# fenghansen/YOND_public

Measured on NVIDIA B200. Metric: raw_MP_per_s_end_to_end_YOND_denoise, higher is better.
Workload: dtype bf16

## Files before the change

yond_public_b200/csrc/conv_tc.cu:

```cuda
#include "conv_tc.cuh"

#include <mutex>

namespace {

constexpr int kEpiWarps = 16;
constexpr int kThreads = 64 + 32 * kEpiWarps;
constexpr int kMaxStagesA = 8;
constexpr int kMaxStagesB = 8;
constexpr int kMaxT = 4;
static_assert(kMaxT == 4, "conv_tc: the issuer dispatches T in {1, 2, 4}");
constexpr int kMaxNT = 256;
constexpr int kCta2MinNT = 128;
constexpr int kMaxTabStages = 64;

struct FastDiv {
  uint32_t mul, shr, d;
};
__host__ FastDiv make_fastdiv(uint32_t d) {
  FastDiv f{0u, 0u, d};
  if (d > 1) {
    uint32_t lg = 0;
    while ((1u << lg) < d) ++lg;
    const uint32_t pw = 31 + lg;
    f.mul = (uint32_t)(((1ull << pw) + d - 1) / d);
    f.shr = pw - 32;
  }
  return f;
}
__device__ __forceinline__ uint32_t fdiv(uint32_t n, const FastDiv& f) { return f.d == 1 ? n : (__umulhi(n, f.mul) >> f.shr); }

struct TcParams {
  int B, H, W;
  int TW, TH, NB, T;
  int t_along_h;
  int tiles_h, tiles_w, tiles_b, tiles_n;
  int NT;
  int N;
  int Cout;
  int CB;
  int ncb0, ncb1;
  int mode;
  int wres;
  int SA, SB;
  uint32_t a_stage_bytes, a_tx_bytes, b_stage_bytes;
  uint32_t sub_off, sbo, tap_r_off;
  uint32_t smem_b_off, smem_bar_off, smem_epi_off;
  int tmem_cols;
  uint32_t b2_stage_bytes, b2_off;
  int cta2;
  int acc_stages;
  FastDiv fd_tiles_n, fd_tiles_w, fd_tiles_h, fd_cout;
  int lg_nchunk;
  uint32_t t_off;
  int epi_split;
  int epi_fixed;
  int paired;
  int cvec;
  uint32_t cmask;
  const float* bias;
  const float* scale;
  const float* shift;
  int act;
  float slope;
  const bf16* res;
  bf16* out0;
  bf16* out1;
  const float* tail_w;
  const float* tail_b;
  const float* tail_z;
  const float* tail_ub;
  float* tail_y;
  int tail_res;
  uint32_t smem_tail_off;
};

struct TcMaps {
  CUtensorMap a[8];
  CUtensorMap w;
  CUtensorMap w2;
};

__device__ __forceinline__ uint32_t smem_u32(const void* p) { return (uint32_t)__cvta_generic_to_shared(p); }

__device__ __forceinline__ void mbar_init(uint32_t bar, uint32_t count) {
  asm volatile("mbarrier.init.shared::cta.b64 [%0], %1;" ::"r"(bar), "r"(count) : "memory");
}
__device__ __forceinline__ void mbar_expect_tx(uint32_t bar, uint32_t bytes) {
  asm volatile("mbarrier.arrive.expect_tx.shared::cta.b64 _, [%0], %1;" ::"r"(bar), "r"(bytes) : "memory");
}
__device__ __forceinline__ void mbar_arrive(uint32_t bar) {
  asm volatile("mbarrier.arrive.shared::cta.b64 _, [%0];" ::"r"(bar) : "memory");
}
__device__ __forceinline__ void mbar_wait(uint32_t bar, uint32_t parity) {
  uint32_t done = 0;
  long long t0 = 0;
  for (uint32_t it = 0;; ++it) {
    asm volatile(
        "{\n\t.reg .pred p;\n\t"
// ... 84 lines not shown
__device__ __forceinline__ void tmem_alloc_pair(uint32_t smem_dst, uint32_t ncols) {
  asm volatile("tcgen05.alloc.cta_group::2.sync.aligned.shared::cta.b32 [%0], %1;" ::"r"(smem_dst), "r"(ncols) : "memory");
}
__device__ __forceinline__ void tmem_relinquish_pair() {
  asm volatile("tcgen05.relinquish_alloc_permit.cta_group::2.sync.aligned;" ::: "memory");
}
__device__ __forceinline__ void tmem_dealloc_pair(uint32_t taddr, uint32_t ncols) {
  asm volatile("tcgen05.dealloc.cta_group::2.sync.aligned.b32 %0, %1;" ::"r"(taddr), "r"(ncols) : "memory");
}
__device__ __forceinline__ void umma_commit_pair(uint32_t bar) {
  asm volatile("tcgen05.commit.cta_group::2.mbarrier::arrive::one.shared::cluster.multicast::cluster.b64 [%0], %1;" ::"r"(bar),
               "h"((uint16_t)3)
               : "memory");
}

__device__ __forceinline__ void tmem_ld16(uint32_t taddr, uint32_t (&v)[16]) {
  asm volatile(
      "tcgen05.ld.sync.aligned.32x32b.x16.b32 "
      "{%0, %1, %2, %3, %4, %5, %6, %7, %8, %9, %10, %11, %12, %13, %14, %15}, [%16];"
      : "=r"(v[0]), "=r"(v[1]), "=r"(v[2]), "=r"(v[3]), "=r"(v[4]), "=r"(v[5]), "=r"(v[6]), "=r"(v[7]), "=r"(v[8]),
        "=r"(v[9]), "=r"(v[10]), "=r"(v[11]), "=r"(v[12]), "=r"(v[13]), "=r"(v[14]), "=r"(v[15])
      : "r"(taddr)
      : "memory");
}
__device__ __forceinline__ void tmem_ld_wait() { asm volatile("tcgen05.wait::ld.sync.aligned;" ::: "memory"); }

__device__ __forceinline__ uint32_t pack_bf16x2(float a, float b) {
  __nv_bfloat162 h = __floats2bfloat162_rn(a, b);
  return *reinterpret_cast<uint32_t*>(&h);
}
__device__ __forceinline__ float2 unpack_bf16x2(uint32_t u) {
  __nv_bfloat162 h = *reinterpret_cast<__nv_bfloat162*>(&u);
  return __bfloat1622float2(h);
}

__device__ __forceinline__ float fast_silu(float v) {
  float t;
  const float h = 0.5f * v;
  asm("tanh.approx.f32 %0, %1;" : "=f"(t) : "f"(h));
  return fmaf(h, t, h);
}

struct AStage {
  int map;
  int c;
  int dw, dh;
  int ntaps;
  int widx0;
  int sx;
};
__device__ __forceinline__ AStage decode_astage(const TcParams& p, int ai) {
  AStage s;
  s.sx = -1;
  if (p.mode == CONV_3X3_S1) {
    const int src = ai >= p.ncb0;
    s.map = src;
    s.c = (src ? ai - p.ncb0 : ai) * p.CB;
    s.dw = -1;
    s.dh = -1;
    s.ntaps = 9;
    s.widx0 = ai * 9;
  } else if (p.mode == CONV_3X3_S2) {
    int cbg = ai / 9, tap = ai - cbg * 9;
    int r = tap / 3, sx = tap - r * 3;
    int src = cbg >= p.ncb0;
    s.map = src * 4 + (r != 1) * 2 + (sx != 1);
    s.c = (src ? cbg - p.ncb0 : cbg) * p.CB;
    s.dh = (r == 0) ? -1 : 0;
    s.dw = (sx == 0) ? -1 : 0;
    s.ntaps = 1;
    s.widx0 = cbg * 9 + tap;
  } else if (p.mode == CONV_UPSC) {
    s.dw = 0;
    s.dh = 0;
    s.ntaps = 1;
    if (ai < p.ncb0) {
      s.map = 0;
      s.c = ai * p.CB;
      s.widx0 = ai;
    } else {
      const int j = ai - p.ncb0;
      const int q = j / p.ncb1, cb = j - q * p.ncb1;
      s.map = 4 + q;
      s.c = cb * p.CB;
      s.widx0 = cb;
      s.sx = q;
    }
  } else {
    int src = ai >= p.ncb0;
    s.map = src;
    s.c = (src ? ai - p.ncb0 : ai) * p.CB;
    s.dw = 0;
    s.dh = 0;
    s.ntaps = 1;
    s.widx0 = ai;
  }
  return s;
}
__host__ __device__ __forceinline__ int num_astages(const TcParams& p) {
  int ncb = p.ncb0 + p.ncb1;
  if (p.mode == CONV_3X3_S1) return ncb;
  if (p.mode == CONV_UPSC) return p.ncb0 + 4 * p.ncb1;
  return p.mode == CONV_3X3_S2 ? ncb * 9 : ncb;
}
__device__ __forceinline__ int num_wtiles(const TcParams& p) {
  int ncb = p.ncb0 + p.ncb1;
  return (p.mode == CONV_3X3_S1 || p.mode == CONV_3X3_S2) ? ncb * 9 : ncb;
}

struct TileCoord {
  int n0, w0, h0, b0, n_idx;
};
__device__ __forceinline__ TileCoord decode_tile(const TcParams& p, int tile) {
  TileCoord t;
  uint32_t m = fdiv((uint32_t)tile, p.fd_tiles_n);
  t.n_idx = tile - (int)m * p.tiles_n;
  uint32_t m2 = fdiv(m, p.fd_tiles_w);
  const int tw_i = (int)(m - m2 * p.tiles_w);
  const uint32_t m3 = fdiv(m2, p.fd_tiles_h);
  const int th_i = (int)(m2 - m3 * p.tiles_h);
  const int tb_i = (int)m3;
  t.w0 = tw_i * p.TW;
  t.h0 = th_i * p.TH * (p.t_along_h ? p.T : 1);
  t.b0 = tb_i * p.NB * (p.t_along_h ? 1 : p.T);
  t.n0 = t.n_idx * p.NT;
  return t;
}

struct TileSched {
  int first, step, n_units, rank, cta2;
};
template <bool kPair>
__device__ __forceinline__ TileSched make_sched(const TcParams& p, int total_tiles) {
  TileSched s;
  s.cta2 = kPair ? 1 : 0;
  if (kPair) {
    s.rank = (int)cluster_ctarank();
    s.first = (int)blockIdx.x >> 1;
    s.step = (int)gridDim.x >> 1;
    const int m_tiles = total_tiles / p.tiles_n;
    s.n_units = ((m_tiles + 1) >> 1) * p.tiles_n;
  } else {
    s.rank = 0;
    s.first = (int)blockIdx.x;
    s.step = (int)gridDim.x;
    s.n_units = total_tiles;
  }
  return s;
}
__device__ __forceinline__ int sched_tile(const TcParams& p, const TileSched& s, int u) {
  if (!s.cta2) return u;
  const int m2 = (int)fdiv((uint32_t)u, p.fd_tiles_n);
  return (2 * m2 + s.rank) * p.tiles_n + (u - m2 * p.tiles_n);
}

__device__ __forceinline__ void umma_step(uint32_t tmem_d, uint32_t& a_lo, uint32_t a_hi, uint32_t& b_lo, uint32_t b_hi,
// ... 37 lines not shown
    dt += nt;
  }
}
template <int KS, int TT>
__device__ __forceinline__ void issue_tap(uint32_t d_tmem, uint32_t nt, uint32_t a_lo0, uint32_t sub_step, uint32_t b_lo0,
                                          uint32_t a_hi, uint32_t b_hi, uint32_t idesc, uint32_t accum) {
  uint32_t al = a_lo0, dt = d_tmem;
#pragma unroll
  for (int t = 0; t < TT; ++t) {
    uint32_t bl = b_lo0;
#pragma unroll
    for (int k = 0; k < KS; ++k) umma_step(dt, al, a_hi, bl, b_hi, idesc, k ? 1u : accum);
    al += sub_step - 2u * KS;
    dt += nt;
  }
}

template <int K0, int K1, int TT>
__device__ __forceinline__ void issue_tap_range(uint32_t d_tmem, uint32_t nt, uint32_t a_lo0, uint32_t sub_step, uint32_t b_lo0,
                                                uint32_t a_hi, uint32_t b_hi, uint32_t idesc, uint32_t accum) {
  uint32_t al = a_lo0 + 2u * K0, dt = d_tmem;
#pragma unroll
  for (int t = 0; t < TT; ++t) {
    uint32_t bl = b_lo0 + 2u * K0;
#pragma unroll
    for (int k = K0; k < K1; ++k) umma_step(dt, al, a_hi, bl, b_hi, idesc, k > K0 ? 1u : accum);
    al += sub_step - 2u * (K1 - K0);
    dt += nt;
  }
}
template <int TT>
__device__ __forceinline__ void issue_slab_paired(uint32_t d_tmem, uint32_t nt, uint32_t a_stage_lo, uint32_t tap_r16, uint32_t px16,
                                                  uint32_t sub_step, uint32_t b_lo_first, uint32_t b_step16, uint32_t a_hi,
                                                  uint32_t b_hi, uint32_t idesc, uint32_t first_accum) {
#pragma unroll
  for (int r = 0; r < 3; ++r) {
    const uint32_t a0 = a_stage_lo + (uint32_t)r * tap_r16, b0 = b_lo_first + (uint32_t)(r * 3) * b_step16;
    issue_tap_range<2, 4, TT>(d_tmem, nt, a0, sub_step, b0, a_hi, b_hi, idesc, r ? 1u : first_accum);
    issue_tap_range<0, 4, TT>(d_tmem, nt, a0 + px16, sub_step, b0 + b_step16, a_hi, b_hi, idesc, 1u);
    issue_tap_range<0, 2, TT>(d_tmem, nt, a0 + 2u * px16, sub_step, b0 + 2u * b_step16, a_hi, b_hi, idesc, 1u);
  }
}

template <int KS, int TT>
__device__ __forceinline__ void issue_slab_resident(uint32_t d_tmem, uint32_t nt, uint32_t a_stage_lo, uint32_t tap_r16, uint32_t px16,
                                                    uint32_t sub_step, uint32_t b_lo_first, uint32_t b_step16, uint32_t a_hi,
                                                    uint32_t b_hi, uint32_t idesc, uint32_t first_accum) {
#pragma unroll
  for (int r = 0; r < 3; ++r)
#pragma unroll
    for (int sx = 0; sx < 3; ++sx)
      issue_tap_range<0, KS, TT>(d_tmem, nt, a_stage_lo + (uint32_t)r * tap_r16 + (uint32_t)sx * px16, sub_step,
                                 b_lo_first + (uint32_t)(r * 3 + sx) * b_step16, a_hi, b_hi, idesc, (r | sx) ? 1u : first_accum);
}

struct __align__(32) U8 { uint32_t v[8]; };
__device__ __forceinline__ void stg256(void* ptr, const U8& u) {
  asm volatile("st.global.v8.b32 [%0], {%1, %2, %3, %4, %5, %6, %7, %8};" ::"l"(ptr), "r"(u.v[0]), "r"(u.v[1]), "r"(u.v[2]), "r"(u.v[3]),
               "r"(u.v[4]), "r"(u.v[5]), "r"(u.v[6]), "r"(u.v[7])
               : "memory");
}
__device__ __forceinline__ U8 ldg256(const void* ptr) {
  U8 u;
  asm volatile("ld.global.nc.v8.b32 {%0, %1, %2, %3, %4, %5, %6, %7}, [%8];"
               : "=r"(u.v[0]), "=r"(u.v[1]), "=r"(u.v[2]), "=r"(u.v[3]), "=r"(u.v[4]), "=r"(u.v[5]), "=r"(u.v[6]), "=r"(u.v[7])
               : "l"(ptr));
  return u;
}

__device__ __forceinline__ float4 lds_f4(uint32_t addr) {
  float4 v;
  asm volatile("ld.shared.v4.f32 {%0, %1, %2, %3}, [%4];" : "=f"(v.x), "=f"(v.y), "=f"(v.z), "=f"(v.w) : "r"(addr) : "memory");
  return v;
}
__device__ __forceinline__ void sts_f32(uint32_t addr, float v) { asm volatile("st.shared.f32 [%0], %1;" ::"r"(addr), "f"(v) : "memory"); }
__device__ __forceinline__ void sts_u4(uint32_t addr, uint32_t a, uint32_t b, uint32_t c, uint32_t d) {
  asm volatile("st.shared.v4.b32 [%0], {%1, %2, %3, %4};" ::"r"(addr), "r"(a), "r"(b), "r"(c), "r"(d) : "memory");
}
__device__ __forceinline__ uint4 lds_u4(uint32_t addr) {
  uint4 v;
  asm volatile("ld.shared.v4.b32 {%0, %1, %2, %3}, [%4];" : "=r"(v.x), "=r"(v.y), "=r"(v.z), "=r"(v.w) : "r"(addr));
  return v;
}

__device__ __forceinline__ bool epilogue_single_set(const TcParams& p) {
  const int nparts = p.epi_split ? 2 : 4, nchunk = 1 << p.lg_nchunk;
  const int nsets = nchunk > nparts ? nchunk / nparts : 1;
  return p.epi_fixed != 0 && nsets <= 2 && (nsets == 1 || (((uint32_t)(nparts << 4) & p.cmask) == 0u));
}
template <bool kScale, bool kRes, bool kSilu, int kV, bool kPair, bool kRegP = false>
__device__ __forceinline__ void epilogue_loop(const TcParams& p, uint32_t tmem_base, uint32_t acc_full, uint32_t acc_empty, uint32_t ptab,
                                              int warp, int lane, int total_tiles) {
  const TileSched sched = make_sched<kPair>(p, total_tiles);
  const uint32_t acc_empty_remote = kPair ? mapa_shared(acc_empty, 0) : acc_empty;
  const int q = warp & 3;
  const int part4 = (warp - 2) >> 2;
  const bool split = p.epi_split != 0;
  const int grp = split ? (part4 & 1) : 0;
  const int part = split ? (part4 >> 1) : part4;
  const int nparts = split ? 2 : 4;
  const int row = q * 32 + lane;
  const int w_i = row & (p.TW - 1);
  const int g_i = row / p.TW;
  const int dh = g_i / p.NB, db = g_i & (p.NB - 1);
  const int nchunk = 1 << p.lg_nchunk, nchunk_m1 = nchunk - 1, nvis = p.T << p.lg_nchunk;
  const int nsets = nchunk > nparts ? nchunk / nparts : 1;
// ... 306 lines not shown
    mbar_init(w_full, 1);
    fence_barrier_init();
  }
  if (p.tail_w) {
    for (int i = threadIdx.x; i < 132; i += blockDim.x)
      sts_f32(smem_base + p.smem_tail_off + 4 * i, i < 128 ? __ldg(p.tail_w + i) : __ldg(p.tail_b + i - 128));
  }
  if (warp == 1) {
    if (kPair) {
      tmem_alloc_pair(tmem_slot, p.tmem_cols);
      tmem_relinquish_pair();
    } else {
      tmem_alloc(tmem_slot, p.tmem_cols);
      tmem_relinquish();
    }
  }
  tc_fence_before();
  __syncthreads();
  if (kPair) cluster_sync_all();
  tc_fence_after();
  const TileSched sched = make_sched<kPair>(p, total_tiles);
  const bool pair_leader = sched.rank == 0;
  uint32_t tmem_base;
  asm volatile("ld.shared.u32 %0, [%1];" : "=r"(tmem_base) : "r"(tmem_slot));

  if (warp == 0) {
    const uint32_t is_leader = elect_one();
    if (is_leader) {
      tma_prefetch_desc(&maps.w);
      tma_prefetch_desc(&maps.a[0]);
      if (p.wres && p.mode == CONV_UPSC) {
        mbar_expect_tx(w_full, p.ncb0 * p.b_stage_bytes + p.ncb1 * p.b2_stage_bytes);
        for (int i = 0; i < p.ncb0; ++i) tma_load_2d(smem_b + i * p.b_stage_bytes, &maps.w, w_full, 0, i * p.N);
        for (int i = 0; i < p.ncb1; ++i) tma_load_2d(smem_b + p.b2_off + i * p.b2_stage_bytes, &maps.w2, w_full, 0, i * p.Cout);
      } else if (p.wres) {
        const int nwt = num_wtiles(p);
        mbar_expect_tx(w_full, nwt * p.b_stage_bytes);
        for (int i = 0; i < nwt; ++i) tma_load_2d(smem_b + i * p.b_stage_bytes, &maps.w, w_full, 0, i * p.N);
      }
    }
    __syncwarp();
    int sa = 0, pa = 0, sb = 0, pb = 0;
    const uint32_t a_full_sig = kPair ? mapa_shared(a_full, 0) : a_full;
    const uint32_t b_full_sig = kPair ? mapa_shared(b_full, 0) : b_full;
    const uint32_t b_half = kPair ? (uint32_t)(sched.rank * (p.NT / 2)) : 0u;
    for (int u = sched.first; u < sched.n_units; u += sched.step) {
      const TileCoord tc = decode_tile(p, sched_tile(p, sched, u));
      for (int ai = 0; ai < n_ast; ++ai) {
        const AStage s = decode_astage(p, ai);
        mbar_wait(a_empty + 8 * sa, pa ^ 1);
        if (is_leader) {
          if (kPair) {
            if (pair_leader) mbar_expect_tx(a_full + 8 * sa, 2 * p.a_tx_bytes);
            tma_load_4d_pair(smem_a + sa * p.a_stage_bytes, &maps.a[s.map], a_full_sig + 8 * sa, s.c, tc.w0 + s.dw, tc.b0, tc.h0 + s.dh);
          } else {
            mbar_expect_tx(a_full + 8 * sa, p.a_tx_bytes);
            tma_load_4d(smem_a + sa * p.a_stage_bytes, &maps.a[s.map], a_full + 8 * sa, s.c, tc.w0 + s.dw, tc.b0, tc.h0 + s.dh);
          }
        }
        __syncwarp();
        if (++sa == p.SA) { sa = 0; pa ^= 1; }
        if (!p.wres) {
          for (int j = 0; j < s.ntaps; ++j) {
            const int widx = s.widx0 + j;
            mbar_wait(b_empty + 8 * sb, pb ^ 1);
            if (is_leader) {
              if (kPair) {
                if (pair_leader) mbar_expect_tx(b_full + 8 * sb, 2 * p.b_stage_bytes);
                tma_load_2d_pair(smem_b + sb * p.b_stage_bytes, &maps.w, b_full_sig + 8 * sb, 0, widx * p.N + tc.n0 + (int)b_half);
              } else {
                mbar_expect_tx(b_full + 8 * sb, p.b_stage_bytes);
                tma_load_2d(smem_b + sb * p.b_stage_bytes, &maps.w, b_full + 8 * sb, 0, widx * p.N + tc.n0);
              }
            }
            __syncwarp();
            if (++sb == p.SB) { sb = 0; pb ^= 1; }
          }
        }
      }
    }
  } else if (warp == 1) {
    const uint32_t u_tmem = __reduce_max_sync(0xffffffffu, tmem_base);
    const uint32_t u_smem_a = __reduce_max_sync(0xffffffffu, smem_a);
    const uint32_t u_smem_b = __reduce_max_sync(0xffffffffu, smem_b);
    const uint32_t u_bars = __reduce_max_sync(0xffffffffu, bars);
    const uint32_t ua_full = u_bars, ua_empty = ua_full + 8 * kMaxStagesA;
    const uint32_t ub_full = ua_empty + 8 * kMaxStagesA, ub_empty = ub_full + 8 * kMaxStagesB;
    const uint32_t uacc_full = ub_empty + 8 * kMaxStagesB, uacc_empty = uacc_full + 16;
    const uint32_t uw_full = uacc_empty + 16;
    const uint32_t idesc = (1u << 4) | (1u << 7) | (1u << 10) | ((uint32_t)(p.NT >> 3) << 17) | (((kPair ? 256u : 128u) >> 4) << 24);
    const uint32_t idesc_full = idesc;
    const int ksteps = p.CB / 16;
    const uint32_t layout = (row_bytes == 128) ? 2u : 4u;
    const uint32_t a_hi = ((p.sbo >> 4) & 0x3FFFu) | (1u << 14) | (layout << 29);
    const uint32_t b_hi = (((8u * row_bytes) >> 4) & 0x3FFFu) | (1u << 14) | (layout << 29);
    const uint32_t lo_flags = 1u << 16;
    const uint32_t sub_step = p.sub_off >> 4;
    const uint32_t tap_r16 = p.tap_r_off >> 4, px16 = row_bytes >> 4;
    const uint32_t nt = (uint32_t)p.NT;
    const bool leader = elect_one() != 0;
    if (p.wres) mbar_wait(uw_full, 0);
    int sa = 0, pa = 0, sb = 0, pb = 0, as = 0, pacc = 0;
    const bool fast_slab1 = p.wres && p.mode == CONV_3X3_S1 && n_ast == 1 && !kPair;
    if (fast_slab1) {
      const uint32_t b_first = (((u_smem_b) & 0x3FFFFu) >> 4) | lo_flags;
      const uint32_t b_step16 = p.b_stage_bytes >> 4;
      const uint32_t a_bytes = p.a_stage_bytes, acc_cols = (uint32_t)p.T * nt;
      const int SA = p.SA, nacc = p.acc_stages;
      auto run = [&](auto issue) {
        for (int u = sched.first; u < sched.n_units; u += sched.step) {
          mbar_wait(uacc_empty + 8 * as, pacc ^ 1);
          mbar_wait(ua_full + 8 * sa, pa);
          tc_fence_after();
          if (leader) {
            issue(u_tmem + (uint32_t)as * acc_cols, (((u_smem_a + (uint32_t)sa * a_bytes) & 0x3FFFFu) >> 4) | lo_flags);
            umma_commit(ua_empty + 8 * sa);
            umma_commit(uacc_full + 8 * as);
          }
          __syncwarp();
          if (++sa == SA) { sa = 0; pa ^= 1; }
          if (++as == nacc) { as = 0; pacc ^= 1; }
        }
      };
#define YOND_SLAB1(FN) run([&](uint32_t d, uint32_t a_lo) { FN(d, nt, a_lo, tap_r16, px16, sub_step, b_first, b_step16, a_hi, b_hi, idesc, 0u); })
      if (p.paired) {
        if (p.T == 1) YOND_SLAB1((issue_slab_paired<1>));
        else if (p.T == 2) YOND_SLAB1((issue_slab_paired<2>));
        else YOND_SLAB1((issue_slab_paired<4>));
      } else if (ksteps == 4) {
        if (p.T == 1) YOND_SLAB1((issue_slab_resident<4, 1>));
        else if (p.T == 2) YOND_SLAB1((issue_slab_resident<4, 2>));
        else YOND_SLAB1((issue_slab_resident<4, 4>));
      } else {
        if (p.T == 1) YOND_SLAB1((issue_slab_resident<2, 1>));
        else if (p.T == 2) YOND_SLAB1((issue_slab_resident<2, 2>));
        else YOND_SLAB1((issue_slab_resident<2, 4>));
      }
#undef YOND_SLAB1
    }
    const bool fast_tab = p.wres && p.mode != CONV_3X3_S1 && !kPair;
    if (fast_tab) {
      const uint32_t tab = smem_base + p.smem_tail_off;
      for (int ai = lane; ai < n_ast; ai += 32) {
        const AStage s = decode_astage(p, ai);
        uint32_t b_lo0 = (((smem_b + (uint32_t)s.widx0 * p.b_stage_bytes) & 0x3FFFFu) >> 4) | lo_flags;
        uint32_t id = idesc_full, d_off = 0;
        if (p.mode == CONV_UPSC && s.sx >= 0) {
          b_lo0 = (((smem_b + p.b2_off + (uint32_t)s.widx0 * p.b2_stage_bytes) & 0x3FFFFu) >> 4) | lo_flags;
          id = (idesc_full & ~(0x3Fu << 17)) | ((uint32_t)(p.Cout >> 3) << 17);
          d_off = (uint32_t)(s.sx * p.Cout);
        }
        sts_u4(tab + 16u * (uint32_t)ai, b_lo0, id, d_off, 0u);
      }
      __syncwarp();
      const uint32_t a_bytes = p.a_stage_bytes, acc_cols = (uint32_t)p.T * nt;
      const int SA = p.SA, nacc = p.acc_stages;
      auto run = [&](auto issue) {
        for (int u = sched.first; u < sched.n_units; u += sched.step) {
          mbar_wait(uacc_empty + 8 * as, pacc ^ 1);
          const uint32_t d_tile = u_tmem + (uint32_t)as * acc_cols;
          for (int ai = 0; ai < n_ast; ++ai) {
            mbar_wait(ua_full + 8 * sa, pa);
            tc_fence_after();
            if (leader) {
              const uint4 e = lds_u4(tab + 16u * (uint32_t)ai);
              issue(d_tile + e.z, (((u_smem_a + (uint32_t)sa * a_bytes) & 0x3FFFFu) >> 4) | lo_flags, e.x, e.y, ai ? 1u : 0u);
              umma_commit(ua_empty + 8 * sa);
            }
            __syncwarp();
            if (++sa == SA) { sa = 0; pa ^= 1; }
          }
          if (leader) umma_commit(uacc_full + 8 * as);
          __syncwarp();
          if (++as == nacc) { as = 0; pacc ^= 1; }
        }
      };
#define YOND_TAB(KS, TT) run([&](uint32_t d, uint32_t a_lo, uint32_t b_lo, uint32_t id, uint32_t acc) { issue_tap<KS, TT>(d, nt, a_lo, sub_step, b_lo, a_hi, b_hi, id, acc); })
      if (ksteps == 4) {
        if (p.T == 1) YOND_TAB(4, 1);
        else if (p.T == 2) YOND_TAB(4, 2);
        else YOND_TAB(4, 4);
      } else {
        if (p.T == 1) YOND_TAB(2, 1);
        else if (p.T == 2) YOND_TAB(2, 2);
        else YOND_TAB(2, 4);
      }
#undef YOND_TAB
    }
    const bool fast_stream = !p.wres && p.mode == CONV_3X3_S1 && ksteps == 4;
    if (fast_stream && (!kPair || pair_leader)) {
      const uint32_t a_bytes = p.a_stage_bytes, b_bytes = p.b_stage_bytes, acc_cols = (uint32_t)p.T * nt;
      const int SA = p.SA, SB = p.SB, nacc = p.acc_stages;
      auto commit = [&](uint32_t bar) {
        if (kPair) umma_commit_pair(bar);
        else umma_commit(bar);
      };
      auto run = [&](auto issue) {
        for (int u = sched.first; u < sched.n_units; u += sched.step) {
          mbar_wait(uacc_empty + 8 * as, pacc ^ 1);
          const uint32_t d_tile = u_tmem + (uint32_t)as * acc_cols;
          for (int ai = 0; ai < n_ast; ++ai) {
            mbar_wait(ua_full + 8 * sa, pa);
            tc_fence_after();
            if (leader) {
              const uint32_t a_stage_lo = (((u_smem_a + (uint32_t)sa * a_bytes) & 0x3FFFFu) >> 4) | lo_flags;
              int lsb = sb, lpb = pb;
#pragma unroll
              for (int j = 0; j < 9; ++j) {
                const uint32_t r = j / 3, sx = j % 3;
                mbar_wait(ub_full + 8 * lsb, lpb);
                tc_fence_after();
                issue(d_tile, a_stage_lo + r * tap_r16 + sx * px16, (((u_smem_b + (uint32_t)lsb * b_bytes) & 0x3FFFFu) >> 4) | lo_flags,
                      (ai | j) ? 1u : 0u);
                commit(ub_empty + 8 * lsb);
                if (++lsb == SB) { lsb = 0; lpb ^= 1; }
              }
              commit(ua_empty + 8 * sa);
            }
            __syncwarp();
            sb += 9;
            while (sb >= SB) { sb -= SB; pb ^= 1; }
            if (++sa == SA) { sa = 0; pa ^= 1; }
          }
          if (leader) commit(uacc_full + 8 * as);
          __syncwarp();
          if (++as == nacc) { as = 0; pacc ^= 1; }
        }
      };
#define YOND_STREAM(TT)                                                                                                   \
  run([&](uint32_t d, uint32_t a_lo, uint32_t b_lo, uint32_t acc) {                                                      \
    if (kPair) issue_tap_pair<4, TT>(d, nt, a_lo, sub_step, b_lo, a_hi, b_hi, idesc, acc);                               \
    else issue_tap<4, TT>(d, nt, a_lo, sub_step, b_lo, a_hi, b_hi, idesc, acc);                                          \
  })
      if (p.T == 1) YOND_STREAM(1);
      else if (p.T == 2) YOND_STREAM(2);
      else YOND_STREAM(4);
#undef YOND_STREAM
    }
    if (!kPair && !fast_slab1 && !fast_tab && !fast_stream) {
      for (int u = sched.first; u < sched.n_units; u += sched.step) {
        mbar_wait(uacc_empty + 8 * as, pacc ^ 1);
        tc_fence_after();
        const uint32_t d_tmem = u_tmem + (uint32_t)(as * p.T) * nt;
        for (int ai = 0; ai < n_ast; ++ai) {
          const AStage s = decode_astage(p, ai);
          mbar_wait(ua_full + 8 * sa, pa);
          tc_fence_after();
          const uint32_t a_stage_lo = (((u_smem_a + (uint32_t)sa * p.a_stage_bytes) & 0x3FFFFu) >> 4) | lo_flags;
          if (leader && p.wres) {
            const uint32_t b_first = (((u_smem_b + (uint32_t)s.widx0 * p.b_stage_bytes) & 0x3FFFFu) >> 4) | lo_flags;
            const uint32_t b_step16 = p.b_stage_bytes >> 4;
            const uint32_t acc0 = ai ? 1u : 0u;
            if (ksteps == 4) {
              if (p.T == 1) issue_slab_resident<4, 1>(d_tmem, nt, a_stage_lo, tap_r16, px16, sub_step, b_first, b_step16, a_hi, b_hi, idesc, acc0);
              else if (p.T == 2) issue_slab_resident<4, 2>(d_tmem, nt, a_stage_lo, tap_r16, px16, sub_step, b_first, b_step16, a_hi, b_hi, idesc, acc0);
              else issue_slab_resident<4, 4>(d_tmem, nt, a_stage_lo, tap_r16, px16, sub_step, b_first, b_step16, a_hi, b_hi, idesc, acc0);
            } else {
              if (p.T == 1) issue_slab_resident<2, 1>(d_tmem, nt, a_stage_lo, tap_r16, px16, sub_step, b_first, b_step16, a_hi, b_hi, idesc, acc0);
              else if (p.T == 2) issue_slab_resident<2, 2>(d_tmem, nt, a_stage_lo, tap_r16, px16, sub_step, b_first, b_step16, a_hi, b_hi, idesc, acc0);
              else issue_slab_resident<2, 4>(d_tmem, nt, a_stage_lo, tap_r16, px16, sub_step, b_first, b_step16, a_hi, b_hi, idesc, acc0);
            }
            umma_commit(ua_empty + 8 * sa);
          } else if (leader) {
            int lsb = sb, lpb = pb;
            for (int j = 0; j < s.ntaps; ++j) {
              uint32_t r = 0, sx = 0;
              if (p.mode == CONV_3X3_S1) { r = (j >= 3) + (j >= 6); sx = j - r * 3; }
              mbar_wait(ub_full + 8 * lsb, lpb);
              tc_fence_after();
              const uint32_t a_lo0 = a_stage_lo + r * tap_r16 + sx * px16;
              const uint32_t b_lo0 = (((u_smem_b + (uint32_t)lsb * p.b_stage_bytes) & 0x3FFFFu) >> 4) | lo_flags;
              const uint32_t accum = (ai | j) ? 1u : 0u;
              if (ksteps == 4) {
                if (p.T == 1) issue_tap<4, 1>(d_tmem, nt, a_lo0, sub_step, b_lo0, a_hi, b_hi, idesc, accum);
                else if (p.T == 2) issue_tap<4, 2>(d_tmem, nt, a_lo0, sub_step, b_lo0, a_hi, b_hi, idesc, accum);
                else issue_tap<4, 4>(d_tmem, nt, a_lo0, sub_step, b_lo0, a_hi, b_hi, idesc, accum);
              } else {
                if (p.T == 1) issue_tap<2, 1>(d_tmem, nt, a_lo0, sub_step, b_lo0, a_hi, b_hi, idesc, accum);
                else if (p.T == 2) issue_tap<2, 2>(d_tmem, nt, a_lo0, sub_step, b_lo0, a_hi, b_hi, idesc, accum);
                else issue_tap<2, 4>(d_tmem, nt, a_lo0, sub_step, b_lo0, a_hi, b_hi, idesc, accum);
              }
              umma_commit(ub_empty + 8 * lsb);
              if (++lsb == p.SB) { lsb = 0; lpb ^= 1; }
            }
            umma_commit(ua_empty + 8 * sa);
          }
          __syncwarp();
          if (!p.wres) {
            sb += s.ntaps;
            while (sb >= p.SB) { sb -= p.SB; pb ^= 1; }
          }
          if (++sa == p.SA) { sa = 0; pa ^= 1; }
        }
        if (leader) umma_commit(uacc_full + 8 * as);
        __syncwarp();
        if (++as == p.acc_stages) { as = 0; pacc ^= 1; }
      }
    }
  } else {
    const bool silu = p.act == ACT_SILU;
    const uint32_t ptab = smem_base + p.smem_epi_off + (uint32_t)(warp - 2) * 256u;
#define YOND_EPI(S, R, A, V) epilogue_loop<S, R, A, V, kPair>(p, tmem_base, acc_full, acc_empty, ptab, warp, lane, total_tiles)
    const bool few = p.T * (p.NT / 16) <= 8;
    if (!kPair && p.tail_w) {
      const uint32_t tailtab = smem_base + p.smem_tail_off;
      if (p.scale && p.res) epilogue_tail<true, true>(p, tmem_base, acc_full, acc_empty, ptab, tailtab, warp, lane, total_tiles);
      else if (p.scale) epilogue_tail<true, false>(p, tmem_base, acc_full, acc_empty, ptab, tailtab, warp, lane, total_tiles);
      else if (p.res) epilogue_tail<false, true>(p, tmem_base, acc_full, acc_empty, ptab, tailtab, warp, lane, total_tiles);
      else epilogue_tail<false, false>(p, tmem_base, acc_full, acc_empty, ptab, tailtab, warp, lane, total_tiles);
    }
    else if (p.scale && p.res) { if (silu) YOND_EPI(true, true, true, 2); else YOND_EPI(true, true, false, 2); }
    else if (p.scale && epilogue_single_set(p)) {
      if (silu) epilogue_loop<true, false, true, 4, kPair, true>(p, tmem_base, acc_full, acc_empty, ptab, warp, lane, total_tiles);
      else epilogue_loop<true, false, false, 4, kPair, true>(p, tmem_base, acc_full, acc_empty, ptab, warp, lane, total_tiles);
    }
    else if (p.scale) { if (silu) YOND_EPI(true, false, true, 4); else YOND_EPI(true, false, false, 4); }
    else if (p.res && epilogue_single_set(p)) {
#define YOND_EPI_R(A, V) epilogue_loop<false, true, A, V, kPair, true>(p, tmem_base, acc_full, acc_empty, ptab, warp, lane, total_tiles)
      if (few) { if (silu) YOND_EPI_R(true, 2); else YOND_EPI_R(false, 2); }
      else { if (silu) YOND_EPI_R(true, 4); else YOND_EPI_R(false, 4); }
#undef YOND_EPI_R
    }
    else if (p.res) {
// ... 89 lines not shown
  for (int r = 0; r < 3; ++r)
    for (int P = -1; P <= 1; ++P)
      for (int o = 0; o < 2; ++o)
        for (int co = 0; co < 32; ++co)
          for (int i = 0; i < 2; ++i)
            for (int ci = 0; ci < 32; ++ci) {
              const int dx = 2 * P + i - o;
              const float v = (dx >= -1 && dx <= 1) ? w[((size_t)co * 32 + ci) * 9 + r * 3 + (dx + 1)] : 0.f;
              out[((size_t)(r * 3 + P + 1) * 64 + (o * 32 + co)) * 64 + (i * 32 + ci)] = __float2bfloat16_rn(v);
            }
}

int conv_tc_launch(const ConvLayer& Lin, cudaStream_t stream) {
  ConvLayer L = Lin;
  const bool paired = L.wpaired && L.mode == CONV_3X3_S1 && L.Cin0 == 32 && L.Cin1 == 0 && L.Cout == 32 && L.Win % 2 == 0 &&
                      L.res == nullptr && L.tail_w == nullptr;
  if (paired) {
    L.Win /= 2;
    L.Cin0 = 64;
    L.Cout = 64;
    L.wpacked = L.wpaired;
  }
  YOND_REQUIRE(L.Cin0 % 32 == 0 && L.Cin1 % 32 == 0 && L.Cin0 > 0, "conv_tc: Cin must be a multiple of 32 (got %d,%d)",
               L.Cin0, L.Cin1);
  YOND_REQUIRE(L.Cout % 32 == 0, "conv_tc: Cout must be a multiple of 32 (got %d)", L.Cout);
  YOND_REQUIRE((double)L.B * L.Hin * L.Win * ((L.mode == CONVT_2X2 || L.mode == CONV_UPSC) ? 4.0 : 1.0) * L.Cout < 4294967296.0,
               "conv_tc: output of %d x %d x %d x %d elements exceeds the 32-bit offset range; split the batch", L.B, L.Hin, L.Win, L.Cout);
  YOND_REQUIRE(L.scale != nullptr || L.shift == nullptr, "conv_tc: a shift vector needs a scale vector");
  TcParams p{};
  p.mode = L.mode;
  p.B = L.B;
  if (L.mode == CONV_3X3_S2) {
    YOND_REQUIRE(L.Hin % 2 == 0 && L.Win % 2 == 0, "conv_tc: stride-2 conv needs even input dims");
    p.H = L.Hin / 2;
    p.W = L.Win / 2;
  } else {
    p.H = L.Hin;
    p.W = L.Win;
  }
  p.Cout = L.Cout;
  p.paired = paired ? 1 : 0;
  p.cvec = paired ? 32 : L.Cout;
  p.cmask = paired ? 31u : 0xffffffffu;
  const bool convt_like = L.mode == CONVT_2X2 || L.mode == CONV_UPSC;
  p.N = convt_like ? 4 * L.Cout : L.Cout;
  p.CB = conv_tc_channel_block(L.Cin0, L.Cin1);
  p.ncb0 = L.Cin0 / p.CB;
  p.ncb1 = L.Cin1 / p.CB;
  p.NT = p.N < kMaxNT ? p.N : kMaxNT;
  YOND_REQUIRE(p.N % p.NT == 0 && (p.NT & (p.NT - 1)) == 0, "conv_tc: unsupported N=%d", p.N);
  p.tiles_n = p.N / p.NT;
  const uint32_t row_bytes = p.CB * 2;
  const bool conv3 = L.mode == CONV_3X3_S1;

  p.TW = conv3 ? 8 : (p.W > 8 ? 16 : 8);
  const int rows = 128 / p.TW;
  p.TH = pow2_ceil(p.H) < rows ? pow2_ceil(p.H) : rows;
  p.NB = rows / p.TH;
  const int ncb = p.ncb0 + p.ncb1;
  const int nwt = ((L.mode == CONV_3X3_S1 || L.mode == CONV_3X3_S2) ? 9 : 1) * ncb;
  const size_t smem_budget = 227 * 1024 - 2048 - kEpiWarps * 256 - 1024;
  p.b_stage_bytes = (uint32_t)p.NT * row_bytes;
  YOND_REQUIRE(p.b_stage_bytes % 1024 == 0, "conv_tc: weight stage not 1024-aligned");
  size_t wres_bytes = (size_t)nwt * p.b_stage_bytes;
  if (L.mode == CONV_UPSC) {
    YOND_REQUIRE(L.Cin1 == L.Cout && L.src1 != nullptr, "conv_tc: fused up-sampling needs a skip source with Cout channels");
    p.b2_stage_bytes = (uint32_t)L.Cout * row_bytes;
    p.b2_off = (uint32_t)p.ncb0 * p.b_stage_bytes;
    wres_bytes = (size_t)p.b2_off + (size_t)p.ncb1 * p.b2_stage_bytes;
    YOND_REQUIRE(p.tiles_n == 1 && wres_bytes <= 80 * 1024 && p.b2_stage_bytes % 1024 == 0,
                 "conv_tc: fused up-sampling is built for resident weights (Cout <= 64); got Cout=%d", L.Cout);
  }
  p.wres = (p.tiles_n == 1 && wres_bytes <= 80 * 1024) ? 1 : 0;
  YOND_REQUIRE(!p.wres || conv3 || num_astages(p) <= kMaxTabStages, "conv_tc: %d resident-weight stages exceed the stage table (%d)",
               num_astages(p), kMaxTabStages);
  p.cta2 = (conv3 && !p.wres && p.CB == 64 && p.NT >= kCta2MinNT && yond_num_sms() >= 2) ? 1 : 0;
  if (p.cta2) p.b_stage_bytes /= 2;
  int T = 1;
  {
    int tmax = (p.wres || p.cta2) ? 512 / (2 * p.NT) : 512 / p.NT;
    if (tmax > kMaxT) tmax = kMaxT;
    if (p.NB == 1) {
      while (T * 2 <= tmax && (p.H >= p.TH * T * 2 || (conv3 && p.B >= T * 2))) T *= 2;
    } else if (conv3) {
      while (T * 2 <= tmax && p.B >= p.NB * T * 2) T *= 2;
    }
  }
  int slab_w = 0, slab_h = 0, SBt = 0;
  size_t b_region = 0;
  for (;; T /= 2) {
    p.T = T;
    p.t_along_h = (p.H >= p.TH * T) ? 1 : 0;
    const int SH = p.TH * (p.t_along_h ? T : 1);
    SBt = p.NB * (p.t_along_h ? 1 : T);
    p.tiles_w = ceil_div(p.W, p.TW);
    p.tiles_h = ceil_div(p.H, SH);
    p.tiles_b = ceil_div(p.B, SBt);
    slab_w = conv3 ? p.TW + 2 : p.TW;
    slab_h = conv3 ? SH + 2 : SH;
    const uint32_t line = (uint32_t)slab_w * row_bytes;
    p.a_tx_bytes = (uint32_t)slab_h * SBt * line;
    p.a_stage_bytes = (uint32_t)align_up((size_t)p.a_tx_bytes, 1024);
    if (conv3) {
      p.tap_r_off = (uint32_t)SBt * line;
      p.sbo = p.t_along_h ? line : (uint32_t)T * line;
      p.sub_off = p.t_along_h ? (uint32_t)p.TH * line : line;
    } else {
      p.tap_r_off = 0;
      p.sbo = 8u * row_bytes;
      p.sub_off = (uint32_t)p.TH * line;
    }
    if (p.wres) {
      p.SB = 1;
      b_region = wres_bytes;
      p.SA = (int)((smem_budget - b_region) / p.a_stage_bytes);
      if (p.SA > kMaxStagesA) p.SA = kMaxStagesA;
      if (p.SA >= 3 || T == 1) break;
    } else {
      const size_t rest = smem_budget > 2 * (size_t)p.a_stage_bytes ? smem_budget - 2 * (size_t)p.a_stage_bytes : 0;
      p.SB = (int)(rest / p.b_stage_bytes);
      if (p.SB > kMaxStagesB) p.SB = kMaxStagesB;
      b_region = (size_t)p.SB * p.b_stage_bytes;
      p.SA = p.SB > 0 ? (int)((smem_budget - b_region) / p.a_stage_bytes) : 0;
      if (p.SA > kMaxStagesA) p.SA = kMaxStagesA;
      if ((p.SB >= 3 && p.SA >= 2) || T == 1) break;
    }
  }
  YOND_REQUIRE(p.SB >= 1, "conv_tc: not enough shared memory for the weight ring");
  YOND_REQUIRE(p.SA >= 2, "conv_tc: not enough shared memory for the activation pipeline");
  p.smem_b_off = (uint32_t)p.SA * p.a_stage_bytes;
  p.smem_bar_off = (uint32_t)align_up(p.smem_b_off + b_region, 1024);
  p.smem_epi_off = p.smem_bar_off + 512;
  p.smem_tail_off = p.smem_epi_off + kEpiWarps * 256;
  const size_t smem_bytes = p.smem_tail_off + 1024 + 1024;
  p.acc_stages = 2 * p.T * p.NT <= 512 ? 2 : 1;
  p.epi_split = (p.acc_stages == 2 && p.paired) ? 1 : 0;
  p.tmem_cols = p.acc_stages * p.T * p.NT < 32 ? 32 : p.acc_stages * p.T * p.NT;
  YOND_REQUIRE(p.tmem_cols <= 512, "conv_tc: TMEM budget exceeded");

  p.fd_tiles_n = make_fastdiv((uint32_t)p.tiles_n);
  p.fd_tiles_w = make_fastdiv((uint32_t)p.tiles_w);
  p.fd_tiles_h = make_fastdiv((uint32_t)p.tiles_h);
  p.fd_cout = make_fastdiv((uint32_t)p.Cout);
  p.lg_nchunk = 0;
  while ((16 << p.lg_nchunk) < p.NT) ++p.lg_nchunk;
  if (convt_like) p.t_off = (uint32_t)p.TH * 4u * p.W * p.Cout;
  else p.t_off = (p.t_along_h ? (uint32_t)p.TH * p.W : (uint32_t)p.H * p.W) * (uint32_t)p.Cout;
  YOND_REQUIRE(L.act != ACT_LRELU || (L.slope >= 0.f && L.slope <= 1.f), "conv_tc: LeakyReLU slope must be in [0, 1]");
  {
    const int nchunk = p.NT / 16;
    p.epi_fixed = (p.tiles_n == 1 && nchunk <= 4 && p.NB == 1 && (p.T == 1 || p.t_along_h) && !convt_like) ? 1 : 0;
  }
  p.bias = L.bias;
  p.scale = L.scale;
  p.shift = L.shift;
  p.act = L.act;
  p.slope = L.slope;
  p.res = L.res;
  p.out0 = L.out0;
  p.out1 = L.out1;
  if (L.tail_w) {
    YOND_REQUIRE(L.mode == CONV_3X3_S1 && L.Cout == 32 && !paired && p.tiles_n == 1 && p.NT == 32 && p.T <= 4 && !p.cta2 && L.tail_b &&
                     L.tail_y && (L.tail_z || !L.tail_res),
                 "conv_tc: the fused output conv needs a 3x3 layer with 32 output channels");
    p.tail_w = L.tail_w;
    p.tail_b = L.tail_b;
    p.tail_z = L.tail_z;
    p.tail_ub = L.tail_ub;
    p.tail_y = L.tail_y;
    p.tail_res = L.tail_res;
    p.epi_split = 0;
  }

  TcMaps maps;
  memset(&maps, 0, sizeof(maps));
  const bf16* srcs[2] = {L.src0, L.src1};
  const int cins[2] = {L.Cin0, L.Cin1};
  for (int s = 0; s < 2; ++s) {
    if (cins[s] == 0) continue;
    const int C = cins[s];
    if (L.mode == CONV_UPSC && s == 1) {
      for (int ph = 0; ph < 2; ++ph)
        for (int pw = 0; pw < 2; ++pw) {
          const int Wh = 2 * L.Win, Hh = 2 * L.Hin;
          const bf16* base = srcs[s] + ((size_t)ph * Wh + pw) * C;
          int rc = make_act_map(&maps.a[4 + ph * 2 + pw], base, C, L.Win, L.B, L.Hin, (uint64_t)2 * C * 2,
                                (uint64_t)Hh * Wh * C * 2, (uint64_t)2 * Wh * C * 2, p.CB, slab_w, SBt, slab_h);
          if (rc) return rc;
        }
    } else if (L.mode == CONV_3X3_S2) {
      for (int ph = 0; ph < 2; ++ph)
        for (int pw = 0; pw < 2; ++pw) {
          const bf16* base = srcs[s] + ((size_t)ph * L.Win + pw) * C;
          int rc = make_act_map(&maps.a[s * 4 + ph * 2 + pw], base, C, L.Win / 2, L.B, L.Hin / 2, (uint64_t)2 * C * 2,
                                (uint64_t)L.Hin * L.Win * C * 2, (uint64_t)2 * L.Win * C * 2, p.CB, slab_w, SBt, slab_h);
          if (rc) return rc;
        }
    } else {
      int rc = make_act_map(&maps.a[s], srcs[s], C, L.Win, L.B, L.Hin, (uint64_t)C * 2, (uint64_t)L.Hin * L.Win * C * 2,
                            (uint64_t)L.Win * C * 2, p.CB, slab_w, SBt, slab_h);
      if (rc) return rc;
    }
  }
  {
    const size_t rows_a = L.mode == CONV_UPSC ? (size_t)p.ncb0 * p.N : (size_t)nwt * p.N;
    int rc = make_weight_map(&maps.w, L.wpacked, p.CB, rows_a, p.cta2 ? p.NT / 2 : p.NT);
    if (rc) return rc;
    if (L.mode == CONV_UPSC) {
      rc = make_weight_map(&maps.w2, L.wpacked + rows_a * p.CB, p.CB, (size_t)p.ncb1 * L.Cout, L.Cout);
      if (rc) return rc;
    }
  }
  static std::once_flag attr_once;
  static cudaError_t attr_err = cudaSuccess;
  std::call_once(attr_once, [] {
    attr_err = cudaFuncSetAttribute(conv_tc_kernel<false>, cudaFuncAttributeMaxDynamicSharedMemorySize, 227 * 1024);
    if (attr_err == cudaSuccess)
      attr_err = cudaFuncSetAttribute(conv_tc_kernel<true>, cudaFuncAttributeMaxDynamicSharedMemorySize, 227 * 1024);
  });
  if (attr_err != cudaSuccess)
    return yond_set_error(YOND_ERR_CUDA, "cudaFuncSetAttribute(conv_tc_kernel) failed: %s", cudaGetErrorString(attr_err));

  const int total_tiles = p.tiles_b * p.tiles_h * p.tiles_w * p.tiles_n;
  if (p.cta2) {
    const int m_tiles = total_tiles / p.tiles_n;
    const int units = ((m_tiles + 1) / 2) * p.tiles_n;
    int grid = yond_num_sms() & ~1;
    if (grid > 2 * units) grid = 2 * units;
    cudaLaunchConfig_t cfg{};
    cfg.gridDim = dim3((unsigned)grid);
    cfg.blockDim = dim3(kThreads);
    cfg.dynamicSmemBytes = smem_bytes;
    cfg.stream = stream;
    cudaLaunchAttribute attr[1];
    attr[0].id = cudaLaunchAttributeClusterDimension;
    attr[0].val.clusterDim.x = 2;
    attr[0].val.clusterDim.y = 1;
    attr[0].val.clusterDim.z = 1;
    cfg.attrs = attr;
    cfg.numAttrs = 1;
    cudaError_t e = cudaLaunchKernelEx(&cfg, conv_tc_kernel<true>, maps, p);
    if (e != cudaSuccess) return yond_set_error(YOND_ERR_CUDA, "conv_tc: cluster launch failed: %s", cudaGetErrorString(e));
    yond_count_launch(1);
    return YOND_OK;
  }
  int grid = yond_num_sms();
  if (grid > total_tiles) grid = total_tiles;
  conv_tc_kernel<false><<<grid, kThreads, smem_bytes, stream>>>(maps, p);
// ... 4 lines not shown
```

Baseline: 2845.

## Load all four stride-2 parity slabs per channel block and issue 9 taps from smem

Stride-2 3x3 convolutions previously used one activation stage per tap, issuing nine separate TMA loads of shifted parity slabs per channel block. Now each A stage holds all four parity sub-slabs (odd-row ones one row taller, with one extra column), and the MMA issuer walks the nine taps through precomputed smem offsets. The S2 path is also routed through the resident-slab, streaming and 2-CTA paths that S1 already used. This cuts TMA traffic and pipeline stages by roughly nine times. In exchange each stage is larger, which means fewer stages fit in shared memory, and the S2 path is forced to T=1.

```diff
diff --git a/yond_public_b200/csrc/conv_tc.cu b/yond_public_b200/csrc/conv_tc.cu
--- a/yond_public_b200/csrc/conv_tc.cu
+++ b/yond_public_b200/csrc/conv_tc.cu
@@ -45,6 +45,7 @@
   int SA, SB;
   uint32_t a_stage_bytes, a_tx_bytes, b_stage_bytes;
   uint32_t sub_off, sbo, tap_r_off;
+  uint32_t par_off[4], s2_tap16[9];
   uint32_t smem_b_off, smem_bar_off, smem_epi_off;
   int tmem_cols;
   uint32_t b2_stage_bytes, b2_off;
@@ -235,24 +236,14 @@
 __device__ __forceinline__ AStage decode_astage(const TcParams& p, int ai) {
   AStage s;
   s.sx = -1;
-  if (p.mode == CONV_3X3_S1) {
+  if (p.mode == CONV_3X3_S1 || p.mode == CONV_3X3_S2) {
     const int src = ai >= p.ncb0;
-    s.map = src;
+    s.map = p.mode == CONV_3X3_S2 ? src * 4 : src;
     s.c = (src ? ai - p.ncb0 : ai) * p.CB;
     s.dw = -1;
     s.dh = -1;
     s.ntaps = 9;
     s.widx0 = ai * 9;
-  } else if (p.mode == CONV_3X3_S2) {
-    int cbg = ai / 9, tap = ai - cbg * 9;
-    int r = tap / 3, sx = tap - r * 3;
-    int src = cbg >= p.ncb0;
-    s.map = src * 4 + (r != 1) * 2 + (sx != 1);
-    s.c = (src ? cbg - p.ncb0 : cbg) * p.CB;
-    s.dh = (r == 0) ? -1 : 0;
-    s.dw = (sx == 0) ? -1 : 0;
-    s.ntaps = 1;
-    s.widx0 = cbg * 9 + tap;
   } else if (p.mode == CONV_UPSC) {
     s.dw = 0;
     s.dh = 0;
@@ -282,9 +273,8 @@
 }
 __host__ __device__ __forceinline__ int num_astages(const TcParams& p) {
   int ncb = p.ncb0 + p.ncb1;
-  if (p.mode == CONV_3X3_S1) return ncb;
   if (p.mode == CONV_UPSC) return p.ncb0 + 4 * p.ncb1;
-  return p.mode == CONV_3X3_S2 ? ncb * 9 : ncb;
+  return ncb;
 }
 __device__ __forceinline__ int num_wtiles(const TcParams& p) {
   int ncb = p.ncb0 + p.ncb1;
@@ -428,6 +418,14 @@
     for (int sx = 0; sx < 3; ++sx)
       issue_tap_range<0, KS, TT>(d_tmem, nt, a_stage_lo + (uint32_t)r * tap_r16 + (uint32_t)sx * px16, sub_step,
                                  b_lo_first + (uint32_t)(r * 3 + sx) * b_step16, a_hi, b_hi, idesc, (r | sx) ? 1u : first_accum);
+}
+template <int KS>
+__device__ __forceinline__ void issue_slab_s2(uint32_t d_tmem, uint32_t a_stage_lo, const uint32_t (&tap16)[9], uint32_t b_lo_first,
+                                              uint32_t b_step16, uint32_t a_hi, uint32_t b_hi, uint32_t idesc, uint32_t first_accum) {
+#pragma unroll
+  for (int j = 0; j < 9; ++j)
+    issue_tap_range<0, KS, 1>(d_tmem, 0u, a_stage_lo + tap16[j], 0u, b_lo_first + (uint32_t)j * b_step16, a_hi, b_hi, idesc,
+                              j ? 1u : first_accum);
 }
 
 struct __align__(32) U8 { uint32_t v[8]; };
@@ -840,10 +838,18 @@
         if (is_leader) {
           if (kPair) {
             if (pair_leader) mbar_expect_tx(a_full + 8 * sa, 2 * p.a_tx_bytes);
-            tma_load_4d_pair(smem_a + sa * p.a_stage_bytes, &maps.a[s.map], a_full_sig + 8 * sa, s.c, tc.w0 + s.dw, tc.b0, tc.h0 + s.dh);
           } else {
             mbar_expect_tx(a_full + 8 * sa, p.a_tx_bytes);
-            tma_load_4d(smem_a + sa * p.a_stage_bytes, &maps.a[s.map], a_full + 8 * sa, s.c, tc.w0 + s.dw, tc.b0, tc.h0 + s.dh);
+          }
+          auto load_a = [&](uint32_t off, int map, int h) {
+            if (kPair) tma_load_4d_pair(smem_a + sa * p.a_stage_bytes + off, &maps.a[map], a_full_sig + 8 * sa, s.c, tc.w0 + s.dw, tc.b0, h);
+            else tma_load_4d(smem_a + sa * p.a_stage_bytes + off, &maps.a[map], a_full + 8 * sa, s.c, tc.w0 + s.dw, tc.b0, h);
+          };
+          if (p.mode == CONV_3X3_S2) {
+#pragma unroll
+            for (int q = 0; q < 4; ++q) load_a(p.par_off[q], s.map + q, tc.h0 + s.dh + 1 - (q >> 1));
+          } else {
+            load_a(0u, s.map, tc.h0 + s.dh);
           }
         }
         __syncwarp();
@@ -889,7 +895,7 @@
     const bool leader = elect_one() != 0;
     if (p.wres) mbar_wait(uw_full, 0);
     int sa = 0, pa = 0, sb = 0, pb = 0, as = 0, pacc = 0;
-    const bool fast_slab1 = p.wres && p.mode == CONV_3X3_S1 && n_ast == 1 && !kPair;
+    const bool fast_slab1 = p.wres && (p.mode == CONV_3X3_S1 || p.mode == CONV_3X3_S2) && n_ast == 1 && !kPair;
     if (fast_slab1) {
       const uint32_t b_first = (((u_smem_b) & 0x3FFFFu) >> 4) | lo_flags;
       const uint32_t b_step16 = p.b_stage_bytes >> 4;
@@ -911,7 +917,10 @@
         }
       };
 #define YOND_SLAB1(FN) run([&](uint32_t d, uint32_t a_lo) { FN(d, nt, a_lo, tap_r16, px16, sub_step, b_first, b_step16, a_hi, b_hi, idesc, 0u); })
-      if (p.paired) {
+      if (p.mode == CONV_3X3_S2) {
+        if (ksteps == 4) run([&](uint32_t d, uint32_t a_lo) { issue_slab_s2<4>(d, a_lo, p.s2_tap16, b_first, b_step16, a_hi, b_hi, idesc, 0u); });
+        else run([&](uint32_t d, uint32_t a_lo) { issue_slab_s2<2>(d, a_lo, p.s2_tap16, b_first, b_step16, a_hi, b_hi, idesc, 0u); });
+      } else if (p.paired) {
         if (p.T == 1) YOND_SLAB1((issue_slab_paired<1>));
         else if (p.T == 2) YOND_SLAB1((issue_slab_paired<2>));
         else YOND_SLAB1((issue_slab_paired<4>));
@@ -926,7 +935,7 @@
       }
 #undef YOND_SLAB1
     }
-    const bool fast_tab = p.wres && p.mode != CONV_3X3_S1 && !kPair;
+    const bool fast_tab = p.wres && p.mode != CONV_3X3_S1 && p.mode != CONV_3X3_S2 && !kPair;
     if (fast_tab) {
       const uint32_t tab = smem_base + p.smem_tail_off;
       for (int ai = lane; ai < n_ast; ai += 32) {
@@ -975,7 +984,7 @@
       }
 #undef YOND_TAB
     }
-    const bool fast_stream = !p.wres && p.mode == CONV_3X3_S1 && ksteps == 4;
+    const bool fast_stream = !p.wres && (p.mode == CONV_3X3_S1 || p.mode == CONV_3X3_S2) && ksteps == 4;
     if (fast_stream && (!kPair || pair_leader)) {
       const uint32_t a_bytes = p.a_stage_bytes, b_bytes = p.b_stage_bytes, acc_cols = (uint32_t)p.T * nt;
       const int SA = p.SA, SB = p.SB, nacc = p.acc_stages;
@@ -983,7 +992,7 @@
         if (kPair) umma_commit_pair(bar);
         else umma_commit(bar);
       };
-      auto run = [&](auto issue) {
+      auto run = [&](auto issue, auto tap_off) {
         for (int u = sched.first; u < sched.n_units; u += sched.step) {
           mbar_wait(uacc_empty + 8 * as, pacc ^ 1);
           const uint32_t d_tile = u_tmem + (uint32_t)as * acc_cols;
@@ -995,10 +1004,9 @@
               int lsb = sb, lpb = pb;
 #pragma unroll
               for (int j = 0; j < 9; ++j) {
-                const uint32_t r = j / 3, sx = j % 3;
                 mbar_wait(ub_full + 8 * lsb, lpb);
                 tc_fence_after();
-                issue(d_tile, a_stage_lo + r * tap_r16 + sx * px16, (((u_smem_b + (uint32_t)lsb * b_bytes) & 0x3FFFFu) >> 4) | lo_flags,
+                issue(d_tile, a_stage_lo + tap_off(j), (((u_smem_b + (uint32_t)lsb * b_bytes) & 0x3FFFFu) >> 4) | lo_flags,
                       (ai | j) ? 1u : 0u);
                 commit(ub_empty + 8 * lsb);
                 if (++lsb == SB) { lsb = 0; lpb ^= 1; }
@@ -1015,14 +1023,16 @@
           if (++as == nacc) { as = 0; pacc ^= 1; }
         }
       };
-#define YOND_STREAM(TT)                                                                                                   \
+      auto s1_tap = [&](int j) { return (uint32_t)(j / 3) * tap_r16 + (uint32_t)(j % 3) * px16; };
+#define YOND_STREAM(TT, TAP)                                                                                              \
   run([&](uint32_t d, uint32_t a_lo, uint32_t b_lo, uint32_t acc) {                                                      \
     if (kPair) issue_tap_pair<4, TT>(d, nt, a_lo, sub_step, b_lo, a_hi, b_hi, idesc, acc);                               \
     else issue_tap<4, TT>(d, nt, a_lo, sub_step, b_lo, a_hi, b_hi, idesc, acc);                                          \
-  })
-      if (p.T == 1) YOND_STREAM(1);
-      else if (p.T == 2) YOND_STREAM(2);
-      else YOND_STREAM(4);
+  }, TAP)
+      if (p.mode == CONV_3X3_S2) YOND_STREAM(1, [&](int j) { return p.s2_tap16[j]; });
+      else if (p.T == 1) YOND_STREAM(1, s1_tap);
+      else if (p.T == 2) YOND_STREAM(2, s1_tap);
+      else YOND_STREAM(4, s1_tap);
 #undef YOND_STREAM
     }
     if (!kPair && !fast_slab1 && !fast_tab && !fast_stream) {
@@ -1039,7 +1049,10 @@
             const uint32_t b_first = (((u_smem_b + (uint32_t)s.widx0 * p.b_stage_bytes) & 0x3FFFFu) >> 4) | lo_flags;
             const uint32_t b_step16 = p.b_stage_bytes >> 4;
             const uint32_t acc0 = ai ? 1u : 0u;
-            if (ksteps == 4) {
+            if (p.mode == CONV_3X3_S2) {
+              if (ksteps == 4) issue_slab_s2<4>(d_tmem, a_stage_lo, p.s2_tap16, b_first, b_step16, a_hi, b_hi, idesc, acc0);
+              else issue_slab_s2<2>(d_tmem, a_stage_lo, p.s2_tap16, b_first, b_step16, a_hi, b_hi, idesc, acc0);
+            } else if (ksteps == 4) {
               if (p.T == 1) issue_slab_resident<4, 1>(d_tmem, nt, a_stage_lo, tap_r16, px16, sub_step, b_first, b_step16, a_hi, b_hi, idesc, acc0);
               else if (p.T == 2) issue_slab_resident<4, 2>(d_tmem, nt, a_stage_lo, tap_r16, px16, sub_step, b_first, b_step16, a_hi, b_hi, idesc, acc0);
               else issue_slab_resident<4, 4>(d_tmem, nt, a_stage_lo, tap_r16, px16, sub_step, b_first, b_step16, a_hi, b_hi, idesc, acc0);
@@ -1052,11 +1065,16 @@
           } else if (leader) {
             int lsb = sb, lpb = pb;
             for (int j = 0; j < s.ntaps; ++j) {
-              uint32_t r = 0, sx = 0;
-              if (p.mode == CONV_3X3_S1) { r = (j >= 3) + (j >= 6); sx = j - r * 3; }
+              uint32_t a_tap = 0;
+              if (p.mode == CONV_3X3_S1) {
+                const uint32_t r = (j >= 3) + (j >= 6), sx = j - r * 3;
+                a_tap = r * tap_r16 + sx * px16;
+              } else if (p.mode == CONV_3X3_S2) {
+                a_tap = p.s2_tap16[j];
+              }
               mbar_wait(ub_full + 8 * lsb, lpb);
               tc_fence_after();
-              const uint32_t a_lo0 = a_stage_lo + r * tap_r16 + sx * px16;
+              const uint32_t a_lo0 = a_stage_lo + a_tap;
               const uint32_t b_lo0 = (((u_smem_b + (uint32_t)lsb * p.b_stage_bytes) & 0x3FFFFu) >> 4) | lo_flags;
               const uint32_t accum = (ai | j) ? 1u : 0u;
               if (ksteps == 4) {
@@ -1252,8 +1270,9 @@
   p.tiles_n = p.N / p.NT;
   const uint32_t row_bytes = p.CB * 2;
   const bool conv3 = L.mode == CONV_3X3_S1;
-
-  p.TW = conv3 ? 8 : (p.W > 8 ? 16 : 8);
+  const bool s2 = L.mode == CONV_3X3_S2;
+
+  p.TW = (conv3 || s2) ? 8 : (p.W > 8 ? 16 : 8);
   const int rows = 128 / p.TW;
   p.TH = pow2_ceil(p.H) < rows ? pow2_ceil(p.H) : rows;
   p.NB = rows / p.TH;
@@ -1272,12 +1291,12 @@
                  "conv_tc: fused up-sampling is built for resident weights (Cout <= 64); got Cout=%d", L.Cout);
   }
   p.wres = (p.tiles_n == 1 && wres_bytes <= 80 * 1024) ? 1 : 0;
-  YOND_REQUIRE(!p.wres || conv3 || num_astages(p) <= kMaxTabStages, "conv_tc: %d resident-weight stages exceed the stage table (%d)",
+  YOND_REQUIRE(!p.wres || conv3 || s2 || num_astages(p) <= kMaxTabStages, "conv_tc: %d resident-weight stages exceed the stage table (%d)",
                num_astages(p), kMaxTabStages);
-  p.cta2 = (conv3 && !p.wres && p.CB == 64 && p.NT >= kCta2MinNT && yond_num_sms() >= 2) ? 1 : 0;
+  p.cta2 = ((conv3 || s2) && !p.wres && p.CB == 64 && p.NT >= kCta2MinNT && yond_num_sms() >= 2) ? 1 : 0;
   if (p.cta2) p.b_stage_bytes /= 2;
   int T = 1;
-  {
+  if (!s2) {
     int tmax = (p.wres || p.cta2) ? 512 / (2 * p.NT) : 512 / p.NT;
     if (tmax > kMaxT) tmax = kMaxT;
     if (p.NB == 1) {
@@ -1296,12 +1315,23 @@
     p.tiles_w = ceil_div(p.W, p.TW);
     p.tiles_h = ceil_div(p.H, SH);
     p.tiles_b = ceil_div(p.B, SBt);
-    slab_w = conv3 ? p.TW + 2 : p.TW;
-    slab_h = conv3 ? SH + 2 : SH;
+    slab_w = conv3 ? p.TW + 2 : s2 ? p.TW + 1 : p.TW;
+    slab_h = conv3 ? SH + 2 : s2 ? SH + 1 : SH;
     const uint32_t line = (uint32_t)slab_w * row_bytes;
-    p.a_tx_bytes = (uint32_t)slab_h * SBt * line;
-    p.a_stage_bytes = (uint32_t)align_up((size_t)p.a_tx_bytes, 1024);
-    if (conv3) {
+    if (s2) {
+      const uint32_t even = (uint32_t)SH * SBt * line, odd = (uint32_t)(SH + 1) * SBt * line;
+      const uint32_t even_al = (uint32_t)align_up(even, 1024), odd_al = (uint32_t)align_up(odd, 1024);
+      p.par_off[0] = 0;
+      p.par_off[1] = even_al;
+      p.par_off[2] = 2 * even_al;
+      p.par_off[3] = 2 * even_al + odd_al;
+      p.a_tx_bytes = 2 * even + 2 * odd;
+      p.a_stage_bytes = 2 * even_al + 2 * odd_al;
+    } else {
+      p.a_tx_bytes = (uint32_t)slab_h * SBt * line;
+      p.a_stage_bytes = (uint32_t)align_up((size_t)p.a_tx_bytes, 1024);
+    }
+    if (conv3 || s2) {
       p.tap_r_off = (uint32_t)SBt * line;
       p.sbo = p.t_along_h ? line : (uint32_t)T * line;
       p.sub_off = p.t_along_h ? (uint32_t)p.TH * line : line;
@@ -1328,6 +1358,11 @@
   }
   YOND_REQUIRE(p.SB >= 1, "conv_tc: not enough shared memory for the weight ring");
   YOND_REQUIRE(p.SA >= 2, "conv_tc: not enough shared memory for the activation pipeline");
+  if (s2) {
+    for (int r = 0; r < 3; ++r)
+      for (int sx = 0; sx < 3; ++sx)
+        p.s2_tap16[r * 3 + sx] = (p.par_off[(r != 1) * 2 + (sx != 1)] + (r == 2 ? p.tap_r_off : 0u) + (sx != 0 ? row_bytes : 0u)) >> 4;
+  }
   p.smem_b_off = (uint32_t)p.SA * p.a_stage_bytes;
   p.smem_bar_off = (uint32_t)align_up(p.smem_b_off + b_region, 1024);
   p.smem_epi_off = p.smem_bar_off + 512;
@@ -1393,7 +1428,7 @@
         for (int pw = 0; pw < 2; ++pw) {
           const bf16* base = srcs[s] + ((size_t)ph * L.Win + pw) * C;
           int rc = make_act_map(&maps.a[s * 4 + ph * 2 + pw], base, C, L.Win / 2, L.B, L.Hin / 2, (uint64_t)2 * C * 2,
-                                (uint64_t)L.Hin * L.Win * C * 2, (uint64_t)2 * L.Win * C * 2, p.CB, slab_w, SBt, slab_h);
+                                (uint64_t)L.Hin * L.Win * C * 2, (uint64_t)2 * L.Win * C * 2, p.CB, slab_w, SBt, slab_h - 1 + ph);
           if (rc) return rc;
         }
     } else {
```

Result: no change. 2859 (median of 6 runs) (+0.5%).
